# hammershock/3dgs-avatar-release

Measured on AMD Instinct MI355X. Metric: render fps (fwd+bwd) @200k Gaussians 1024x1024 SH3, higher is better.
Workload: dtype f32; 1 GPU; config3: 200k Gaussians, 1024x1024, SH deg 3, forward+backward; shs+scales+rotations inputs, L1 loss (L1 fused into the rasterizer: l1_target); tile_rect=1, l1=fused, long_lists=0, gaussians=200000, width=1024, height=1024, sh_degree=3, frames_per_rank=1857, total_frames=1857, ranks=1, backend=none, parallelism=frames sharded x1

## Files before the change

3dgs-avatar-release_amd/csrc/capi.hip:

```cpp
#include "common.h"
#include <string.h>
#include <stdlib.h>
#include <atomic>

static thread_local int g_last_hip = 0;
static thread_local const char* g_last_stage = "";
void gs_set_error(int hip_err, const char* stage) {
    g_last_hip = hip_err;
    g_last_stage = stage;
}

static std::atomic<int> g_tune[GS_TUNE_COUNT] = {};
static bool g_tune_init = false;
static void tune_defaults() {
    if (g_tune_init) return;
    g_tune_init = true;
    g_tune[GS_TUNE_XCD_MAP].store(1);
    g_tune[GS_TUNE_DEPTH_SORT].store(1);
    g_tune[GS_TUNE_NT_STORES].store(1);
    g_tune[GS_TUNE_BWD_CHUNKS].store(1);
    g_tune[GS_TUNE_FWD4].store(1);
    if (const char* e = getenv("GSPLAT_FWD4")) g_tune[GS_TUNE_FWD4].store(atoi(e));
    g_tune[GS_TUNE_FWDC_CH].store((int)FWDC_CH_MIN);
    g_tune[GS_TUNE_FWDC_DIV].store((int)FWD4_TOTAL_DIV);
    if (const char* e = getenv("GSPLAT_FWDC_DIV")) { const int v = atoi(e); if (v >= 1) g_tune[GS_TUNE_FWDC_DIV].store(v); }
    if (const char* e = getenv("GSPLAT_FWDC_CH")) { const int v = atoi(e); if (v >= 64 && (v & (v - 1)) == 0) g_tune[GS_TUNE_FWDC_CH].store(v); }
    g_tune[GS_TUNE_SHARED_QLIST].store(1);
    g_tune[GS_TUNE_ONES_FAST].store(1);
    g_tune[GS_TUNE_SMALL_TILES].store(BWD_CHUNK_MAX_TILES);
    g_tune[GS_TUNE_BWD_ORDER].store(1);
    g_tune[GS_TUNE_FWD_MARKS].store(1);
}
int gs_tune_get(int key) {
    tune_defaults();
    return (key >= 0 && key < GS_TUNE_COUNT) ? g_tune[key].load(std::memory_order_relaxed) : 0;
}

#include <vector>
struct ProfRec { const char* name; hipEvent_t a, b; };
struct ProfState {
    bool on = false;
// ... 158 lines not shown

static int forward_phase1(const GsFwdArgs* a, void* geom, size_t geom_bytes, void* img, size_t img_bytes, int32_t* radii,
                          int64_t* count_host_pinned, unsigned long long* poll, void* stream) {
    int rc = validate(a);
    if (rc != GS_OK) return rc;
    if (!geom || !img || (a->P > 0 && !radii)) return GS_E_BAD_ARG;
    const GeomLayout L = geom_layout(a->P);
    const ImgLayout I = img_layout(a->W, a->H, a->long_lists);
    if (geom_bytes < L.total || img_bytes < I.total) return GS_E_WORKSPACE;
    hipStream_t s = (hipStream_t)stream;
    char* g = (char*)geom;
    unsigned long long* count = (unsigned long long*)(g + L.count);
    if (a->P == 0) {
        rc = gs_zero_async(count, 24, "count.zero", s);
        if (rc != GS_OK) return rc;
    } else {
        uint32_t* k0 = (uint32_t*)(g + L.key0);
        uint32_t* k1 = (uint32_t*)(g + L.key1);
        uint32_t* v0 = (uint32_t*)(g + L.val0);
        uint32_t* v1 = (uint32_t*)(g + L.val1);
        ZeroJob zt;
        sort_totals_region((uint32_t*)(g + L.hist), a->P, 32, &zt.ptr, &zt.words);
        const ZeroJob zi{(uint32_t*)((char*)img + I.tile_tot), (int)(I.tile_zero_bytes / 4)};
        { StageScope sc_("preprocess", s);
        rc = launch_preprocess(*a, (float*)(g + L.rec), (float*)(g + L.depths), (uint32_t*)(g + L.tiles),
                               (uint32_t*)(g + L.clamped), k0, v0, radii, (uint32_t*)(g + L.wsum), (uint32_t*)(g + L.wkmin),
                               (uint32_t*)(g + L.wkmax), zt, zi, s); }
        if (rc != GS_OK) return rc;
        if (gs_tune_get(GS_TUNE_DEPTH_SORT)) {
            StageScope sc_("depth_sort", s);
            const DepthSortState st{(unsigned long long*)(g + L.ds_tmp), (unsigned long long*)(g + L.ds_tmp2),
                                    (uint32_t*)(g + L.ds_cnt), (uint32_t*)(g + L.ds_pre),
                                    (uint32_t*)(g + L.ds_tot),
                                    (uint32_t*)(g + L.ds_loc), (uint32_t*)(g + L.ds_grp), (uint32_t*)(g + L.ds_range), L.ds_nb,
                                    L.ds_blocks};
            const PairNumbering pn{(const uint32_t*)(g + L.tiles), (const uint32_t*)(g + L.wsum), (float*)(g + L.rec), count, poll,
                                   (uint32_t*)(g + L.chunk_pairs), (a->P + 255) / 256};
            const RankOut ro{(const float*)(g + L.rec), (const uint32_t*)(g + L.tiles), v0, (uint4*)(g + L.ranklist),
                             (uint32_t*)(g + L.chunk_pairs)};
            rc = launch_depth_sort(k0, (const uint32_t*)(g + L.wkmin), (const uint32_t*)(g + L.wkmax), L.nwaves, a->P, st, pn, ro,
                                   a->debug, s);
            if (rc != GS_OK) return rc;
        } else {
            { StageScope sc_("pair_scan", s);
            rc = launch_first_pair((const uint32_t*)(g + L.tiles), (const uint32_t*)(g + L.wsum), (float*)(g + L.rec), count, poll,
                                   a->P, a->debug, s); }
            if (rc != GS_OK) return rc;
            { StageScope sc_("depth_sort", s);
            rc = launch_sort_pairs(k0, v0, k1, v1, (uint32_t*)(g + L.hist), a->P, 32, true, a->debug, s); }
            if (rc != GS_OK) return rc;
            { StageScope sc_("rank_list", s);
            rc = launch_rank_list(v0, (const float*)(g + L.rec), (const uint32_t*)(g + L.tiles), (uint4*)(g + L.ranklist),
                                  (uint32_t*)(g + L.chunk_pairs), a->P, a->debug, s); }
            if (rc != GS_OK) return rc;
        }
    }
    if (count_host_pinned && (!poll || a->P == 0)) {
        hipError_t e = hipMemcpyAsync(count_host_pinned, count, 8, hipMemcpyDeviceToHost, s);
// ... 616 lines not shown
int gs_tuning(const char* name, int value) {
    if (!name) return GS_E_BAD_ARG;
    tune_defaults();
    if (strcmp(name, "xcd_map") == 0) { g_tune[GS_TUNE_XCD_MAP].store(value); return GS_OK; }
    if (strcmp(name, "small_tiles") == 0) { g_tune[GS_TUNE_SMALL_TILES].store(value); return GS_OK; }
    if (strcmp(name, "ones_fast") == 0) { g_tune[GS_TUNE_ONES_FAST].store(value); return GS_OK; }
    if (strcmp(name, "shared_qlist") == 0) { g_tune[GS_TUNE_SHARED_QLIST].store(value); return GS_OK; }
    if (strcmp(name, "fwd4") == 0) { g_tune[GS_TUNE_FWD4].store(value); return GS_OK; }
    if (strcmp(name, "fwdc_div") == 0) {
        if (value < 1) return GS_E_BAD_ARG;
        g_tune[GS_TUNE_FWDC_DIV].store(value);
        return GS_OK;
    }
    if (strcmp(name, "fwdc_ch") == 0) {
        if (value < 64 || (value & (value - 1)) != 0) return GS_E_BAD_ARG;
        g_tune[GS_TUNE_FWDC_CH].store(value);
        return GS_OK;
    }
    if (strcmp(name, "bwd_chunks") == 0) { g_tune[GS_TUNE_BWD_CHUNKS].store(value); return GS_OK; }
    if (strcmp(name, "nt_stores") == 0) { g_tune[GS_TUNE_NT_STORES].store(value); return GS_OK; }
    if (strcmp(name, "fwd_marks") == 0) { g_tune[GS_TUNE_FWD_MARKS].store(value); return GS_OK; }
    if (strcmp(name, "bwd_order") == 0) { g_tune[GS_TUNE_BWD_ORDER].store(value); return GS_OK; }
    if (strcmp(name, "depth_sort") == 0) { g_tune[GS_TUNE_DEPTH_SORT].store(value); return GS_OK; }
    return GS_E_BAD_ARG;
}

const char* gs_status_string(int code) {
    switch (code) {
        case GS_OK: return "ok";
        case GS_E_BAD_ARG: return "bad argument (null required pointer, non-positive size, unsupported SH degree / more than 16 SH coefficients, or rotations not 16-byte aligned)";
        case GS_E_EXCLUSIVE: return "provide exactly one of shs/colors_precomp and exactly one of (scales, rotations)/cov3D_precomp";
        case GS_E_TOO_LARGE: return "num_rendered or tile grid exceeds the supported index space";
        case GS_E_HIP: return "HIP error";
        case GS_E_WORKSPACE: return "state/workspace buffer smaller than gs_*_bytes requires";
        case GS_E_CAPTURE: return "the stream is being captured into a graph and this call is not capture-safe with these arguments (include/gsplat_mi355.h, \"Stream capture\"); nothing was enqueued";
        default: return "unknown status";
    }
}
int gs_last_hip_error(void) { return g_last_hip; }
const char* gs_last_stage(void) { return g_last_stage; }
const char* gs_build_info(void) { return "gsplat_mi355 gfx950 wave64 tile16 rec48"; }

}
```

3dgs-avatar-release_amd/csrc/common.h:

```cpp
#pragma once
#include <hip/hip_runtime.h>
#include <stdint.h>
#include <stddef.h>
#include "../../include/gsplat_mi355.h"

#define TILE 16
#define WAVE 64
#define REC_F 12
#define GS_MAX_PAIRS 0x3FFFFFFFll

static inline size_t align_up(size_t x, size_t a) { return (x + a - 1) / a * a; }

#define SORT_ITEMS 4096
#define SORT_SMALL_N (1 << 20)
#define SORT_TOTALS_REPL 16
static inline size_t sort_table_words(size_t n) {
    const size_t items = n <= (size_t)SORT_SMALL_N ? 1024 : SORT_ITEMS;
    return (size_t)256 * ((n + items - 1) / items + 4 * SORT_TOTALS_REPL);
}
#define SCAN_ITEMS 2048

#ifndef DS_ITEMS
#define DS_ITEMS 2048
#endif
#ifndef DS_PER_BUCKET
#define DS_PER_BUCKET 64
#endif
static inline int ds_buckets(int P) {
    int nb = (P / DS_PER_BUCKET + 63) / 64 * 64;
    return nb < 256 ? 256 : (nb > 4096 ? 4096 : nb);
}

#define TB_MAX_SEG 64
struct GeomLayout {
    size_t rec, depths, tiles, clamped, key0, key1, val0, val1, ranklist, chunk_pairs, wsum, wkmin, wkmax, hist, count,
        ds_tmp, ds_tmp2, ds_cnt, ds_pre, ds_tot, ds_loc, ds_grp, ds_range, seg_start, total;
    int nblk_sort, nwaves, ds_nb, ds_blocks;
};
static inline GeomLayout geom_layout(int P) {
    GeomLayout L;
    size_t o = 0;
    size_t n = (size_t)(P > 0 ? P : 1);
    auto take = [&](size_t bytes) { size_t at = o; o = align_up(o + bytes, 256); return at; };
    L.nblk_sort = (int)((n + SORT_ITEMS - 1) / SORT_ITEMS);
    L.nwaves = (int)((n + 255) / 256) * 4;
    L.rec = take(n * REC_F * 4);
    L.depths = take(n * 4);
    L.tiles = take(n * 4);
    L.clamped = take(n * 4);
    L.key0 = take(n * 4);
    L.key1 = take(n * 4);
    L.val0 = take(n * 4);
    L.val1 = take(n * 4);
    L.ranklist = take(n * 16);
    L.chunk_pairs = take(((n + 255) / 256) * 4);
    L.wsum = take((size_t)L.nwaves * 4);
    L.wkmin = take((size_t)L.nwaves * 4);
    L.wkmax = take((size_t)L.nwaves * 4);
    L.hist = take(sort_table_words(n) * 4);
    L.count = take(64);
    L.ds_nb = ds_buckets(P);
    L.ds_blocks = (int)((n + DS_ITEMS - 1) / DS_ITEMS);
    L.ds_tmp = take(n * 8);
    L.ds_tmp2 = take(n * 8);
    L.ds_cnt = take((size_t)L.ds_blocks * (L.ds_nb + 1) * 4);
    L.ds_pre = take((size_t)L.ds_blocks * (L.ds_nb + 1) * 4);
    L.ds_tot = take((size_t)(L.ds_nb + 1) * 4);
    L.ds_loc = take((size_t)(L.ds_nb + 1) * 4);
    L.ds_grp = take((size_t)((L.ds_nb + 1 + 63) / 64) * 4);
    L.ds_range = take(16);
    L.seg_start = take((size_t)(TB_MAX_SEG + 2) * 4);
    L.total = o;
    return L;
}

struct BinLayout {
    size_t point_list, qlist, marks, marks_flag, total;
};
static inline BinLayout bin_layout(int64_t D) {
    BinLayout L;
    size_t o = 0;
    size_t n = (size_t)(D > 0 ? D : 1);
    auto take = [&](size_t bytes) { size_t at = o; o = align_up(o + bytes, 256); return at; };
    L.point_list = take(n * 4);
    L.qlist = take(n * 16);
    L.marks = take(n * 16);
    L.marks_flag = take(4);
    L.total = o;
    return L;
}

#define TB_W 64
#ifndef TB_H
#define TB_H 4
#endif
#define TB_TILES (TB_W * TB_H)
struct BinGrid { int nbx, nby, nblocks, nseg_max; };
static inline BinGrid bin_grid(int gx, int gy) {
    BinGrid G;
    G.nbx = (gx + TB_W - 1) / TB_W;
    G.nby = (gy + TB_H - 1) / TB_H;
    G.nblocks = G.nbx * G.nby;
#ifndef TB_TARGET_WGS
#define TB_TARGET_WGS 512
#endif
    int s = (TB_TARGET_WGS + G.nblocks - 1) / G.nblocks;
    G.nseg_max = s < 1 ? 1 : (s > TB_MAX_SEG ? TB_MAX_SEG : s);
    return G;
}
static inline int bin_segments(const BinGrid& G, int P) {
    int s = (P + 1023) / 1024;
    if (s < 1) s = 1;
    return s < G.nseg_max ? s : G.nseg_max;
}

enum { GS_TUNE_XCD_MAP = 0, GS_TUNE_DEPTH_SORT = 1, GS_TUNE_NT_STORES = 2, GS_TUNE_BWD_CHUNKS = 3, GS_TUNE_FWD4 = 4, GS_TUNE_SMALL_TILES = 5, GS_TUNE_SHARED_QLIST = 6, GS_TUNE_ONES_FAST = 7, GS_TUNE_BWD_ORDER = 8, GS_TUNE_FWD_MARKS = 9, GS_TUNE_FWDC_CH = 10, GS_TUNE_FWDC_DIV = 11, GS_TUNE_COUNT = 12 };
int gs_tune_get(int key);

#define BWD_CH 128
#define BWD_KMAX 16
#define BWD_CHUNK_MAX_TILES 2048
#define FWD4_MAX_TILES 2048
#define FWD4_MIN_LIST 512u
#ifndef FWD4_TOTAL_DIV
#define FWD4_TOTAL_DIV 320ull
#endif

#define FWDC_CH_MIN 256u
#define FWDC_SPARSE_PAIRS 524288ull
#define FWDC_MAX_UNITS 4096
#define FWDC_MAX_TILES (FWDC_MAX_UNITS / 2)
#ifdef FWDC_PROF
#define FWDC_SLOTS 9
#else
#define FWDC_SLOTS 8
#endif
#define FWDC_DEAD 0x80000000u
#define FWDC_SPIN_MAX (1 << 16)
struct ImgLayout {
// ... 159 lines not shown
        for (int k = 0; k < 4; k++) {
            const int c = c0 + k0 + k;
            if (k0 + k < per && c < nchunks) {
                const int sgc = segment_of(before, scale, nseg);
                for (int sg = prev_seg + 1; sg <= sgc; sg++) seg_start[sg] = (uint32_t)c;
                prev_seg = sgc;
                before += w[k];
                if (c == nchunks - 1)
                    for (int sg = prev_seg + 1; sg <= nseg; sg++) seg_start[sg] = (uint32_t)nchunks;
            }
        }
    }
}

__device__ __forceinline__ uint32_t xcc_id() {
    uint32_t v;
    asm volatile("s_getreg_b32 %0, hwreg(HW_REG_XCC_ID, 0, 4)" : "=s"(v));
    return v & 7u;
}
__device__ __forceinline__ void zero_job(const ZeroJob z) {
    for (int k = blockIdx.x * blockDim.x + threadIdx.x; k < z.words; k += gridDim.x * blockDim.x) z.ptr[k] = 0u;
}

struct PairCount { const unsigned long long* dev; uint32_t cap; };
__device__ __forceinline__ uint32_t pair_count(const PairCount pc) {
    const unsigned long long d = *pc.dev;
    return d <= (unsigned long long)pc.cap ? (uint32_t)d : 0u;
}


__device__ __forceinline__ void render_block_map(int b, int xmap, int* slot, int* q) {
    if (xmap) {
        *slot = ((b >> 5) << 3) + (b & 7);
        *q = (b >> 3) & 3;
    } else {
        *slot = b >> 2;
        *q = b & 3;
    }
}
static inline bool forward_small_image(int ntiles, int long_lists) { return few_long_lists_mode(ntiles, long_lists) && gs_tune_get(GS_TUNE_FWD4) == 1; }
static inline bool forward_chunked(int ntiles, int long_lists) { return few_long_lists_mode(ntiles, long_lists) && gs_tune_get(GS_TUNE_FWD4) == 2; }
static inline int render_grid_blocks(int ntiles, int xmap) { return xmap ? ((ntiles + 7) / 8) * 32 : ntiles * 4; }

struct StageScope {
    hipStream_t s;
    StageScope(const char* stage, hipStream_t st) : s(st) { gs_prof_begin(stage, st); }
    ~StageScope() { gs_prof_end(s); }
};

int launch_preprocess(const GsFwdArgs& a, float* rec, float* depths, uint32_t* tiles, uint32_t* clamped,
                      uint32_t* sort_keys, uint32_t* sort_vals, int32_t* radii, uint32_t* wave_tiles, uint32_t* wave_kmin,
                      uint32_t* wave_kmax, ZeroJob zero, ZeroJob zero2, hipStream_t s);
struct DepthSortState { unsigned long long *tmp, *tmp2; uint32_t *cnt, *pre, *tot, *loc, *grp, *range; int nb, blocks; };
struct PairNumbering { const uint32_t *tiles, *wave_tiles; float* rec; unsigned long long *count, *host_count; uint32_t* chunk_pairs; int nchunks; };
struct RankOut { const float* rec; const uint32_t* tiles; uint32_t* sorted_idx; uint4* ranklist; uint32_t* chunk_pairs; };
int launch_depth_sort(const uint32_t* keys, const uint32_t* wave_kmin, const uint32_t* wave_kmax, int nwaves, int P,
                      DepthSortState st, PairNumbering pn, RankOut ro, int debug, hipStream_t s);
struct CopyJob { const uint32_t* src; uint32_t* dst; int words; };
struct SecondOnes {
    const float* src_final_T; const uint32_t* src_n_contrib; const uint32_t* src_ncon_c; const uint32_t* src_qcount;
    const float4* src_ckpt; const uint32_t* src_ck_start;
    float* out_color; float* final_T; uint32_t* n_contrib; uint32_t* ncon_c; uint32_t* qcount; float4* ckpt; uint32_t* ck_start;
    const float* bg; int W, H, gx, ntiles, chunks;
};
__device__ __forceinline__ void second_ones_body(const SecondOnes& A, const int block, const int pixel_blocks) {
    if (block < pixel_blocks) {
        const size_t HW = (size_t)A.H * A.W, pid = (size_t)block * 256 + threadIdx.x;
        if (pid < HW) {
            const float Tf = A.src_final_T[pid];
            A.final_T[pid] = Tf;
            A.n_contrib[pid] = A.src_n_contrib[pid];
            A.ncon_c[pid] = A.src_ncon_c[pid];
            A.out_color[pid] = (1.0f - Tf) + Tf * A.bg[0];
            A.out_color[HW + pid] = (1.0f - Tf) + Tf * A.bg[1];
            A.out_color[2 * HW + pid] = (1.0f - Tf) + Tf * A.bg[2];
        }
// ... 148 lines not shown
```

3dgs-avatar-release_amd/csrc/depth_sort.hip:

```cpp
#include "common.h"

#define DS_THREADS 256
#define DS_WAVE_CAP 1024
#define DS_WG_BUCKETS 4
#define DS_CAP_BIG (DS_WG_BUCKETS * DS_WAVE_CAP)

__device__ __forceinline__ unsigned long long ds_bucket_scale(unsigned long long span, int nb) {
    return ((unsigned long long)nb << 32) / span;
}
__device__ __forceinline__ uint32_t ds_bucket_of(uint32_t key, uint32_t kmin, unsigned long long scale, int nb) {
    if (key == 0xFFFFFFFFu || key < kmin) return (uint32_t)nb;
    const uint32_t d = key - kmin;
    const uint32_t lo = (uint32_t)scale, hi = (uint32_t)(scale >> 32);
    const uint32_t b = __umulhi(d, lo) + d * hi;
    return b < (uint32_t)nb ? b : (uint32_t)(nb - 1);
}

#define DS_WAVE_WORDS 16
__global__ __launch_bounds__(DS_THREADS) void ds_count_kernel(const uint32_t* __restrict__ keys,
                                                              const uint32_t* __restrict__ wave_kmin,
                                                              const uint32_t* __restrict__ wave_kmax, int nwaves, int P,
                                                              int nb, uint32_t* __restrict__ cnt,
                                                              uint32_t* __restrict__ krange, const PairNumbering pn) {
    extern __shared__ uint32_t s_hist[];
    __shared__ uint32_t s_red[8];
    __shared__ unsigned long long s_before[DS_THREADS / 64];
    __shared__ uint32_t s_wave[DS_ITEMS / 64 + 1];
    const int tid = threadIdx.x, lane = tid & 63, wid = tid >> 6;
    constexpr int WPB = DS_ITEMS / 64;
    constexpr int NU = DS_ITEMS / DS_THREADS;
    static_assert(WPB <= 64, "one wave scans the workgroup's wave sums");
    static_assert(DS_THREADS == 256, "four partial sums");
    const int w0 = WPB * (int)blockIdx.x;
    const uint32_t* __restrict__ tiles = pn.tiles;
    const uint32_t* __restrict__ wave_tiles = pn.wave_tiles;
    uint32_t k[NU], tv[NU];
#pragma unroll
    for (int u = 0; u < NU; u++) {
        const int i = blockIdx.x * DS_ITEMS + u * DS_THREADS + tid;
        k[u] = i < P ? keys[i] : 0u;
        tv[u] = i < P ? tiles[i] : 0u;
    }
    const uint32_t own = (wid == 0 && lane < WPB && w0 + lane < nwaves) ? wave_tiles[w0 + lane] : 0u;
    uint32_t lo = 0xFFFFFFFFu, hi = 0u;
    unsigned long long before = 0;
    for (int base = 0; base < nwaves; base += DS_THREADS * DS_WAVE_WORDS) {
        uint32_t a[DS_WAVE_WORDS], c[DS_WAVE_WORDS], t[DS_WAVE_WORDS];
#pragma unroll
        for (int u = 0; u < DS_WAVE_WORDS; u++) {
            const int w = base + u * DS_THREADS + tid;
            a[u] = w < nwaves ? wave_kmin[w] : 0xFFFFFFFFu;
            c[u] = w < nwaves ? wave_kmax[w] : 0u;
            t[u] = w < w0 ? wave_tiles[w] : 0u;
        }
#pragma unroll
        for (int u = 0; u < DS_WAVE_WORDS; u++) {
            lo = min(lo, a[u]);
            hi = max(hi, c[u]);
            before += t[u];
        }
    }
    for (int c = blockIdx.x * DS_THREADS + tid; c < pn.nchunks; c += gridDim.x * DS_THREADS) pn.chunk_pairs[c] = 0u;
    for (int b = tid; b <= nb; b += DS_THREADS) s_hist[b] = 0u;
    lo = wave_min(lo);
    hi = wave_max(hi);
    before = wave_sum(before);
    if (lane == 0) { s_red[wid] = lo; s_red[4 + wid] = hi; s_before[wid] = before; }
    if (wid == 0) {
        const uint32_t x = wave_scan_incl(own);
        if (lane < WPB) s_wave[lane] = x - own;
        if (lane == 63) s_wave[WPB] = x;
    }
    __syncthreads();
    const uint32_t kmin = min(min(s_red[0], s_red[1]), min(s_red[2], s_red[3]));
    const uint32_t kmax = max(max(s_red[4], s_red[5]), max(s_red[6], s_red[7]));
    const unsigned long long span = kmax >= kmin ? (unsigned long long)(kmax - kmin) + 1ull : 1ull;
    const unsigned long long block_base = (s_before[0] + s_before[1]) + (s_before[2] + s_before[3]);
    const unsigned long long scale = ds_bucket_scale(span, nb);
    if (blockIdx.x == 0 && tid == 0) {
        krange[0] = kmin;
        krange[1] = (uint32_t)scale;
        krange[2] = (uint32_t)(scale >> 32);
    }
    if (blockIdx.x == gridDim.x - 1 && tid == 0) {
        const unsigned long long total = block_base + s_wave[WPB];
        pn.count[0] = total;
        pn.count[2] = 0ull;
        if (pn.host_count) __hip_atomic_store(pn.host_count, total, __ATOMIC_RELAXED, __HIP_MEMORY_SCOPE_SYSTEM);
    }
#pragma unroll
    for (int u = 0; u < NU; u++) {
        const int i = blockIdx.x * DS_ITEMS + u * DS_THREADS + tid;
        const uint32_t x = wave_scan_incl(tv[u]);
        if (i < P) {
            pn.rec[(size_t)i * REC_F + 9] = __uint_as_float((uint32_t)block_base + s_wave[u * (DS_THREADS / 64) + wid] + x - tv[u]);
            atomicAdd(&s_hist[ds_bucket_of(k[u], kmin, scale, nb)], 1u);
        }
    }
    __syncthreads();
    for (int b = tid; b <= nb; b += DS_THREADS) cnt[(size_t)blockIdx.x * (nb + 1) + b] = s_hist[b];
}

#define DSP_ROWS 32
__global__ __launch_bounds__(256) void ds_prefix_kernel(const uint32_t* __restrict__ cnt, uint32_t* __restrict__ pre,
                                                        uint32_t* __restrict__ tot, uint32_t* __restrict__ loc,
                                                        uint32_t* __restrict__ grp, int nbp, int blocks) {
    __shared__ uint32_t s_part[4][64];
    const int lane = threadIdx.x & 63, wid = threadIdx.x >> 6;
    const int b = blockIdx.x * 64 + lane;
    const bool live = b < nbp;
    const int per = (blocks + 3) >> 2, r0 = wid * per, r1 = min(blocks, r0 + per);
    const bool one_trip = per <= DSP_ROWS;
    uint32_t v[DSP_ROWS];
    uint32_t sum = 0;
    for (int g0 = r0; g0 < r1; g0 += DSP_ROWS) {
#pragma unroll
        for (int u = 0; u < DSP_ROWS; u++) v[u] = (live && g0 + u < r1) ? cnt[(size_t)(g0 + u) * nbp + b] : 0u;
#pragma unroll
        for (int u = 0; u < DSP_ROWS; u++) sum += v[u];
    }
    s_part[wid][lane] = sum;
    __syncthreads();
    uint32_t acc = 0, total = 0;
#pragma unroll
    for (int w = 0; w < 4; w++) {
        const uint32_t q = s_part[w][lane];
        if (w < wid) acc += q;
        total += q;
    }
    for (int g0 = r0; g0 < r1; g0 += DSP_ROWS) {
        if (!one_trip) {
#pragma unroll
            for (int u = 0; u < DSP_ROWS; u++) v[u] = (live && g0 + u < r1) ? cnt[(size_t)(g0 + u) * nbp + b] : 0u;
        }
#pragma unroll
        for (int u = 0; u < DSP_ROWS; u++) {
            if (live && g0 + u < r1) pre[(size_t)(g0 + u) * nbp + b] = acc;
            acc += v[u];
        }
    }
    if (wid == 0) {
        if (live) tot[b] = total;
        const uint32_t x = wave_scan_incl(live ? total : 0u);
        if (live) loc[b] = x - total;
        if (lane == 63) grp[blockIdx.x] = x;
    }
}

#define DS_MAX_NBP 4097
__global__ __launch_bounds__(DS_THREADS) void ds_scatter_kernel(const uint32_t* __restrict__ keys,
                                                                const uint32_t* __restrict__ krange, int P,
                                                                int nb, const uint32_t* __restrict__ cnt,
                                                                const uint32_t* __restrict__ loc,
                                                                const uint32_t* __restrict__ grp,
                                                                unsigned long long* __restrict__ tmp) {
    extern __shared__ uint32_t s_mem[];
    const int nbp = nb + 1;
    uint32_t* s_next = s_mem;
    uint32_t* s_grp = s_mem + nbp;
    const int tid = threadIdx.x;
    constexpr int NB_T = (DS_MAX_NBP + DS_THREADS - 1) / DS_THREADS;
    uint32_t k[DS_ITEMS / DS_THREADS], first[NB_T];
#pragma unroll
    for (int u = 0; u < DS_ITEMS / DS_THREADS; u++) {
        const int i = blockIdx.x * DS_ITEMS + u * DS_THREADS + tid;
        k[u] = i < P ? keys[i] : 0u;
    }
#pragma unroll
    for (int u = 0; u < NB_T; u++) {
        const int b = u * DS_THREADS + tid;
        first[u] = b < nbp ? loc[b] + cnt[(size_t)blockIdx.x * nbp + b] : 0u;
    }
    const int ngrp = (nbp + 63) / 64;
    if (tid < 64) {
        uint32_t x = 0, carry = 0;
        for (int g0 = 0; g0 < ngrp; g0 += 64) {
            const uint32_t v = g0 + tid < ngrp ? grp[g0 + tid] : 0u;
            x = wave_scan_incl(v);
            if (g0 + tid < ngrp) s_grp[g0 + tid] = carry + x - v;
            carry += (uint32_t)__builtin_amdgcn_readlane((int)x, 63);
        }
    }
    const uint32_t kmin = krange[0];
    const unsigned long long scale = (unsigned long long)krange[1] | ((unsigned long long)krange[2] << 32);
    __syncthreads();
#pragma unroll
    for (int u = 0; u < NB_T; u++) {
        const int b = u * DS_THREADS + tid;
        if (b < nbp) s_next[b] = s_grp[b >> 6] + first[u];
    }
    __syncthreads();
#pragma unroll
    for (int u = 0; u < DS_ITEMS / DS_THREADS; u++) {
        const int i = blockIdx.x * DS_ITEMS + u * DS_THREADS + tid;
        if (i < P) {
            const uint32_t pos = atomicAdd(&s_next[ds_bucket_of(k[u], kmin, scale, nb)], 1u);
            tmp[pos] = ((unsigned long long)k[u] << 32) | (unsigned long long)(uint32_t)i;
        }
    }
}

template <typename LOAD, typename STORE, typename SYNC>
__device__ __forceinline__ void ds_bitonic(const long long n, LOAD load, STORE store, SYNC sync) {
    long long n_pad = 2;
    while (n_pad < n) n_pad <<= 1;
    const long long half = n_pad >> 1;
    for (long long k = 2, lk = 0; k <= n_pad; k <<= 1, lk++) {
        for (long long t = threadIdx.x; t < half; t += DS_THREADS) {
            const long long blk = t >> lk, off = t & ((k >> 1) - 1);
            const long long i = blk * k + off, p = blk * k + (k - 1 - off);
            if (p < n) {
                const unsigned long long a = load(i), c = load(p);
                if (a > c) { store(i, c); store(p, a); }
            }
        }
        sync();
        for (long long j = k >> 2; j > 0; j >>= 1) {
            for (long long t = threadIdx.x; t < half; t += DS_THREADS) {
                const long long i = ((t & ~(j - 1)) << 1) | (t & (j - 1)), p = i + j;
// ... 256 lines not shown
        start = wave_sum(part) + in_group;
    }
    const bool large = n > DS_WAVE_CAP;
    if (lane == 0) {
        s_large[wid][0] = large ? (uint32_t)n : 0u;
        s_large[wid][1] = start;
    }
    if (n > 0 && !large) ds_wave_bucket(tmp + start, s + wid * DS_WAVE_CAP, n, start, ro);
    __syncthreads();
    for (int w = 0; w < DS_WG_BUCKETS; w++) {
        const int nl = (int)s_large[w][0];
        if (nl) {
            if (nl > DS_CAP_BIG) ds_giant_bucket(tmp + s_large[w][1], tmp2 + s_large[w][1], s, s_sub, nl, s_large[w][1], ro);
            else ds_large_bucket(tmp + s_large[w][1], s, nl, s_large[w][1], ro);
            __syncthreads();
        }
    }
}

int launch_depth_sort(const uint32_t* keys, const uint32_t* wave_kmin, const uint32_t* wave_kmax, int nwaves, int P,
                      DepthSortState st, PairNumbering pn, RankOut ro, int debug, hipStream_t s) {
    const int nbp = st.nb + 1;
    if (nbp > DS_MAX_NBP) return GS_E_BAD_ARG;
    const size_t lds_count = (size_t)nbp * 4, lds_scatter = (size_t)(nbp + 66) * 4;
    hipLaunchKernelGGL(ds_count_kernel, dim3(st.blocks), dim3(DS_THREADS), lds_count, s, keys, wave_kmin, wave_kmax, nwaves, P,
                       st.nb, st.cnt, st.range, pn);
    GS_LAUNCH_CHECK("depth_sort.count", debug, s);
    hipLaunchKernelGGL(ds_prefix_kernel, dim3((nbp + 63) / 64), dim3(256), 0, s, st.cnt, st.pre, st.tot, st.loc, st.grp, nbp,
                       st.blocks);
    GS_LAUNCH_CHECK("depth_sort.prefix", debug, s);
    hipLaunchKernelGGL(ds_scatter_kernel, dim3(st.blocks), dim3(DS_THREADS), lds_scatter, s, keys, st.range, P, st.nb, st.pre,
                       st.loc, st.grp, st.tmp);
    GS_LAUNCH_CHECK("depth_sort.scatter", debug, s);
    const int helpers = P / 4096 < 1 ? 1 : (P / 4096 > 128 ? 128 : P / 4096);
    hipLaunchKernelGGL(ds_bucket_sort_kernel, dim3((st.nb + DS_WG_BUCKETS - 1) / DS_WG_BUCKETS + helpers), dim3(DS_THREADS), 0, s,
                       st.tmp, st.tmp2, st.tot, st.loc, st.grp, st.nb, ro);
    GS_LAUNCH_CHECK("depth_sort.buckets", debug, s);
    return GS_OK;
}
```

3dgs-avatar-release_amd/csrc/preprocess.hip:

```cpp
#include "common.h"
#include "gs_math.h"

__device__ __forceinline__ float3 load_and_eval_sh(int deg, int M, const float3 p, const float3 campos,
                                                   const float* __restrict__ shs, int i, uint32_t* clamped) {
    const float* g = shs + (size_t)i * M * 3;
    if (M == 16 && ((uintptr_t)shs & 15u) == 0) {
        float l[48];
        const float4* g4 = reinterpret_cast<const float4*>(g);
#pragma unroll
        for (int k = 0; k < 12; k++) {
            const float4 v = g4[k];
            l[4 * k] = v.x; l[4 * k + 1] = v.y; l[4 * k + 2] = v.z; l[4 * k + 3] = v.w;
        }
        return sh_to_rgb(deg, p, campos, l, clamped);
    }
    return sh_to_rgb(deg, p, campos, g, clamped);
}

__global__ __launch_bounds__(256) void preprocess_kernel(
    int P, int deg, int M, const float* __restrict__ means3D, const float* __restrict__ scales,
    float scale_modifier, const float* __restrict__ rotations, const float* __restrict__ opacities,
    const float* __restrict__ shs, const float* __restrict__ colors_precomp, const float* __restrict__ cov3D_precomp,
    const float* __restrict__ viewmatrix, const float* __restrict__ projmatrix, const float* __restrict__ campos,
    int W, int H, float tanfovx, float tanfovy, float focal_x, float focal_y, int gx, int gy, int tile_rect,
    float* __restrict__ rec, float* __restrict__ depths, uint32_t* __restrict__ tiles, uint32_t* __restrict__ clamped,
    uint32_t* __restrict__ sort_keys, uint32_t* __restrict__ sort_vals, int32_t* __restrict__ radii,
    uint32_t* __restrict__ wave_tiles, uint32_t* __restrict__ wave_kmin, uint32_t* __restrict__ wave_kmax, ZeroJob zero,
    ZeroJob zero2) {
    zero_job(zero);
    zero_job(zero2);
    const int gi = blockIdx.x * blockDim.x + threadIdx.x;
    const bool live = gi < P;
    const int i = live ? gi : P - 1;

    float V[16], PV[16];
#pragma unroll
    for (int k = 0; k < 16; k++) { V[k] = viewmatrix[k]; PV[k] = projmatrix[k]; }

    float4 r0 = make_float4(0.f, 0.f, 0.f, 0.f), r1 = r0;
    float r2x = 0.f;
    uint32_t off_bits = 0, rmin_bits = 0, rsize_bits = 0, cl = 0, tt = 0;
    float depth = 0.f;
    int radius = 0;

    const float3 p = make_float3(means3D[3 * i], means3D[3 * i + 1], means3D[3 * i + 2]);
    float c6in[6] = {0.f, 0.f, 0.f, 0.f, 0.f, 0.f};
    float3 sc_in = make_float3(0.f, 0.f, 0.f);
    float4 q_in = make_float4(1.f, 0.f, 0.f, 0.f);
    if (cov3D_precomp) {
#pragma unroll
        for (int k = 0; k < 6; k++) c6in[k] = cov3D_precomp[6 * i + k];
// ... 84 lines not shown
    if (live) {
        float4* R = reinterpret_cast<float4*>(rec) + (size_t)i * 3;
        R[0] = r0;
        R[1] = r1;
        R[2] = make_float4(r2x, __uint_as_float(off_bits), __uint_as_float(rmin_bits), __uint_as_float(rsize_bits));
        depths[i] = depth;
        tiles[i] = tt;
        clamped[i] = cl;
        radii[i] = radius;
        sort_keys[i] = tt ? __float_as_uint(depth) : 0xFFFFFFFFu;
        sort_vals[i] = (uint32_t)i;
    }
    uint32_t wsum = live ? tt : 0u;
    const bool keyed = live && tt != 0u;
    uint32_t kmin = keyed ? __float_as_uint(depth) : 0xFFFFFFFFu, kmax = keyed ? __float_as_uint(depth) : 0u;
    wsum = wave_sum(wsum);
    kmin = wave_min(kmin);
    kmax = wave_max(kmax);
    if ((threadIdx.x & 63) == 0) {
        wave_tiles[gi >> 6] = wsum;
        wave_kmin[gi >> 6] = kmin;
        wave_kmax[gi >> 6] = kmax;
    }
}

int launch_preprocess(const GsFwdArgs& a, float* rec, float* depths, uint32_t* tiles, uint32_t* clamped,
                      uint32_t* sort_keys, uint32_t* sort_vals, int32_t* radii, uint32_t* wave_tiles, uint32_t* wave_kmin,
                      uint32_t* wave_kmax, ZeroJob zero, ZeroJob zero2, hipStream_t s) {
    const int gx = (a.W + TILE - 1) / TILE, gy = (a.H + TILE - 1) / TILE;
    const float focal_y = a.H / (2.0f * a.tanfovy), focal_x = a.W / (2.0f * a.tanfovx);
    const int blocks = (a.P + 255) / 256;
    hipLaunchKernelGGL(preprocess_kernel, dim3(blocks), dim3(256), 0, s, a.P, a.sh_degree, a.M, a.means3D, a.scales,
                       a.scale_modifier, a.rotations, a.opacities, a.shs, a.colors_precomp, a.cov3D_precomp,
                       a.viewmatrix, a.projmatrix, a.campos, a.W, a.H, a.tanfovx, a.tanfovy, focal_x, focal_y, gx, gy,
                       a.tile_rect,
                       rec, depths, tiles, clamped, sort_keys, sort_vals, radii, wave_tiles, wave_kmin, wave_kmax, zero, zero2);
    GS_LAUNCH_CHECK("preprocess", a.debug, s);
    return GS_OK;
}

__global__ __launch_bounds__(256) void recolor_kernel(int P, int deg, int M, const float* __restrict__ means3D,
                                                      const float* __restrict__ shs,
                                                      const float* __restrict__ colors_precomp,
                                                      const float* __restrict__ campos,
                                                      const float4* __restrict__ rec_src,
                                                      const uint32_t* __restrict__ tiles_src,
                                                      float4* __restrict__ rec_dst, uint32_t* __restrict__ tiles_dst,
                                                      uint32_t* __restrict__ clamped_dst,
                                                      unsigned long long* __restrict__ not_ones, const CopyJob c0,
                                                      const CopyJob c1, const ZeroJob z0, const int recolor_blocks, const SecondOnes ones,
                                                      const int pixel_blocks) {
    if ((int)blockIdx.x >= recolor_blocks) {
        second_ones_body(ones, (int)blockIdx.x - recolor_blocks, pixel_blocks);
        return;
    }
    const int i = blockIdx.x * blockDim.x + threadIdx.x;
    for (int k = i; k < c0.words; k += recolor_blocks * (int)blockDim.x) c0.dst[k] = c0.src[k];
    for (int k = i; k < c1.words; k += recolor_blocks * (int)blockDim.x) c1.dst[k] = c1.src[k];
    for (int k = i; k < z0.words; k += recolor_blocks * (int)blockDim.x) z0.ptr[k] = 0u;
// ... 62 lines not shown
```

Baseline: 1720 frames/s.

## Fuse depth-sort bucket counting into preprocess using previous frame's key range

Removes the separate depth-sort count kernel. Preprocess now builds each block's bucket histogram in shared memory, using the depth range stored from the previous call (validated by a tag, padded, with a fixed fallback range). The per-row pair bases and the global key range are computed by an extra block of the prefix kernel, and per-Gaussian pair numbering moves into the scatter kernel. Preprocess blocks grow to DS_ITEMS (now 1024) threads so each block maps to one count row. This saves a launch and a read pass over the keys, but bucket balance now depends on the previous frame's range, and the larger blocks may change occupancy.

```diff
diff --git a/3dgs-avatar-release_amd/csrc/capi.hip b/3dgs-avatar-release_amd/csrc/capi.hip
--- a/3dgs-avatar-release_amd/csrc/capi.hip
+++ b/3dgs-avatar-release_amd/csrc/capi.hip
@@ -17,6 +17,8 @@
     g_tune_init = true;
     g_tune[GS_TUNE_XCD_MAP].store(1);
     g_tune[GS_TUNE_DEPTH_SORT].store(1);
+    g_tune[GS_TUNE_DS_MAP].store(1);
+    if (const char* e = getenv("GSPLAT_DS_MAP")) g_tune[GS_TUNE_DS_MAP].store(atoi(e));
     g_tune[GS_TUNE_NT_STORES].store(1);
     g_tune[GS_TUNE_BWD_CHUNKS].store(1);
     g_tune[GS_TUNE_FWD4].store(1);
@@ -221,18 +223,21 @@
         ZeroJob zt;
         sort_totals_region((uint32_t*)(g + L.hist), a->P, 32, &zt.ptr, &zt.words);
         const ZeroJob zi{(uint32_t*)((char*)img + I.tile_tot), (int)(I.tile_zero_bytes / 4)};
+        const bool bucket_sort = gs_tune_get(GS_TUNE_DEPTH_SORT) != 0;
+        const DsCount dc{(uint32_t*)(g + L.ds_range), bucket_sort ? (uint32_t*)(g + L.ds_cnt) : nullptr, L.ds_nb,
+                         gs_tune_get(GS_TUNE_DS_MAP) == 0 ? 1 : 0};
         { StageScope sc_("preprocess", s);
         rc = launch_preprocess(*a, (float*)(g + L.rec), (float*)(g + L.depths), (uint32_t*)(g + L.tiles),
                                (uint32_t*)(g + L.clamped), k0, v0, radii, (uint32_t*)(g + L.wsum), (uint32_t*)(g + L.wkmin),
-                               (uint32_t*)(g + L.wkmax), zt, zi, s); }
+                               (uint32_t*)(g + L.wkmax), zt, zi, dc, s); }
         if (rc != GS_OK) return rc;
-        if (gs_tune_get(GS_TUNE_DEPTH_SORT)) {
+        if (bucket_sort) {
             StageScope sc_("depth_sort", s);
             const DepthSortState st{(unsigned long long*)(g + L.ds_tmp), (unsigned long long*)(g + L.ds_tmp2),
                                     (uint32_t*)(g + L.ds_cnt), (uint32_t*)(g + L.ds_pre),
                                     (uint32_t*)(g + L.ds_tot),
-                                    (uint32_t*)(g + L.ds_loc), (uint32_t*)(g + L.ds_grp), (uint32_t*)(g + L.ds_range), L.ds_nb,
-                                    L.ds_blocks};
+                                    (uint32_t*)(g + L.ds_loc), (uint32_t*)(g + L.ds_grp), (uint32_t*)(g + L.ds_range),
+                                    (uint32_t*)(g + L.ds_base), L.ds_nb, L.ds_blocks};
             const PairNumbering pn{(const uint32_t*)(g + L.tiles), (const uint32_t*)(g + L.wsum), (float*)(g + L.rec), count, poll,
                                    (uint32_t*)(g + L.chunk_pairs), (a->P + 255) / 256};
             const RankOut ro{(const float*)(g + L.rec), (const uint32_t*)(g + L.tiles), v0, (uint4*)(g + L.ranklist),
@@ -895,6 +900,7 @@
     if (strcmp(name, "fwd_marks") == 0) { g_tune[GS_TUNE_FWD_MARKS].store(value); return GS_OK; }
     if (strcmp(name, "bwd_order") == 0) { g_tune[GS_TUNE_BWD_ORDER].store(value); return GS_OK; }
     if (strcmp(name, "depth_sort") == 0) { g_tune[GS_TUNE_DEPTH_SORT].store(value); return GS_OK; }
+    if (strcmp(name, "ds_map") == 0) { g_tune[GS_TUNE_DS_MAP].store(value); return GS_OK; }
     return GS_E_BAD_ARG;
 }
 
diff --git a/3dgs-avatar-release_amd/csrc/common.h b/3dgs-avatar-release_amd/csrc/common.h
--- a/3dgs-avatar-release_amd/csrc/common.h
+++ b/3dgs-avatar-release_amd/csrc/common.h
@@ -21,7 +21,7 @@
 #define SCAN_ITEMS 2048
 
 #ifndef DS_ITEMS
-#define DS_ITEMS 2048
+#define DS_ITEMS 1024
 #endif
 #ifndef DS_PER_BUCKET
 #define DS_PER_BUCKET 64
@@ -34,7 +34,7 @@
 #define TB_MAX_SEG 64
 struct GeomLayout {
     size_t rec, depths, tiles, clamped, key0, key1, val0, val1, ranklist, chunk_pairs, wsum, wkmin, wkmax, hist, count,
-        ds_tmp, ds_tmp2, ds_cnt, ds_pre, ds_tot, ds_loc, ds_grp, ds_range, seg_start, total;
+        ds_tmp, ds_tmp2, ds_cnt, ds_pre, ds_tot, ds_loc, ds_grp, ds_range, ds_base, seg_start, total;
     int nblk_sort, nwaves, ds_nb, ds_blocks;
 };
 static inline GeomLayout geom_layout(int P) {
@@ -43,7 +43,7 @@
     size_t n = (size_t)(P > 0 ? P : 1);
     auto take = [&](size_t bytes) { size_t at = o; o = align_up(o + bytes, 256); return at; };
     L.nblk_sort = (int)((n + SORT_ITEMS - 1) / SORT_ITEMS);
-    L.nwaves = (int)((n + 255) / 256) * 4;
+    L.nwaves = (int)((n + DS_ITEMS - 1) / DS_ITEMS) * (DS_ITEMS / 64);
     L.rec = take(n * REC_F * 4);
     L.depths = take(n * 4);
     L.tiles = take(n * 4);
@@ -68,7 +68,8 @@
     L.ds_tot = take((size_t)(L.ds_nb + 1) * 4);
     L.ds_loc = take((size_t)(L.ds_nb + 1) * 4);
     L.ds_grp = take((size_t)((L.ds_nb + 1 + 63) / 64) * 4);
-    L.ds_range = take(16);
+    L.ds_range = take(32);
+    L.ds_base = take((size_t)L.ds_blocks * 4);
     L.seg_start = take((size_t)(TB_MAX_SEG + 2) * 4);
     L.total = o;
     return L;
@@ -114,7 +115,7 @@
     return s < G.nseg_max ? s : G.nseg_max;
 }
 
-enum { GS_TUNE_XCD_MAP = 0, GS_TUNE_DEPTH_SORT = 1, GS_TUNE_NT_STORES = 2, GS_TUNE_BWD_CHUNKS = 3, GS_TUNE_FWD4 = 4, GS_TUNE_SMALL_TILES = 5, GS_TUNE_SHARED_QLIST = 6, GS_TUNE_ONES_FAST = 7, GS_TUNE_BWD_ORDER = 8, GS_TUNE_FWD_MARKS = 9, GS_TUNE_FWDC_CH = 10, GS_TUNE_FWDC_DIV = 11, GS_TUNE_COUNT = 12 };
+enum { GS_TUNE_XCD_MAP = 0, GS_TUNE_DEPTH_SORT = 1, GS_TUNE_NT_STORES = 2, GS_TUNE_BWD_CHUNKS = 3, GS_TUNE_FWD4 = 4, GS_TUNE_SMALL_TILES = 5, GS_TUNE_SHARED_QLIST = 6, GS_TUNE_ONES_FAST = 7, GS_TUNE_BWD_ORDER = 8, GS_TUNE_FWD_MARKS = 9, GS_TUNE_FWDC_CH = 10, GS_TUNE_FWDC_DIV = 11, GS_TUNE_DS_MAP = 12, GS_TUNE_COUNT = 13 };
 int gs_tune_get(int key);
 
 #define BWD_CH 128
@@ -320,6 +321,33 @@
     for (int k = blockIdx.x * blockDim.x + threadIdx.x; k < z.words; k += gridDim.x * blockDim.x) z.ptr[k] = 0u;
 }
 
+#define DS_PAD_SHIFT 5
+#define DS_RANGE_TAG 0x6b5d3a17u
+#define DS_FIXED_KMIN 0x3E4CCCCDu
+#define DS_FIXED_KMAX 0x454CCCCDu
+struct DsMap { uint32_t kmin, kmax; unsigned long long scale; };
+__device__ __forceinline__ DsMap ds_map_make(uint32_t kmin, uint32_t kmax, int nb) {
+    DsMap m;
+    m.kmin = kmin;
+    m.kmax = kmax;
+    m.scale = ((unsigned long long)nb << 32) / ((unsigned long long)(kmax - kmin) + 1ull);
+    return m;
+}
+__device__ __forceinline__ DsMap ds_map_stored(uint32_t lo, uint32_t hi, uint32_t tag, int nb, bool fixed) {
+    if (fixed || lo > hi || tag != (lo ^ hi ^ DS_RANGE_TAG)) return ds_map_make(DS_FIXED_KMIN, DS_FIXED_KMAX, nb);
+    const uint32_t pad = (hi - lo) >> DS_PAD_SHIFT;
+    return ds_map_make(lo > pad ? lo - pad : 0u, hi < 0xFFFFFFFFu - pad ? hi + pad : 0xFFFFFFFFu, nb);
+}
+__device__ __forceinline__ uint32_t ds_bucket_of(uint32_t key, const DsMap& m, int nb) {
+    if (key == 0xFFFFFFFFu) return (uint32_t)nb;
+    if (key <= m.kmin) return 0u;
+    if (key >= m.kmax) return (uint32_t)(nb - 1);
+    const uint32_t d = key - m.kmin;
+    const uint32_t lo = (uint32_t)m.scale, hi = (uint32_t)(m.scale >> 32);
+    const uint32_t b = __umulhi(d, lo) + d * hi;
+    return b < (uint32_t)nb ? b : (uint32_t)(nb - 1);
+}
+
 struct PairCount { const unsigned long long* dev; uint32_t cap; };
 __device__ __forceinline__ uint32_t pair_count(const PairCount pc) {
     const unsigned long long d = *pc.dev;
@@ -346,10 +374,11 @@
     ~StageScope() { gs_prof_end(s); }
 };
 
+struct DsCount { uint32_t* range; uint32_t* cnt; int nb, fixed_map; };
 int launch_preprocess(const GsFwdArgs& a, float* rec, float* depths, uint32_t* tiles, uint32_t* clamped,
                       uint32_t* sort_keys, uint32_t* sort_vals, int32_t* radii, uint32_t* wave_tiles, uint32_t* wave_kmin,
-                      uint32_t* wave_kmax, ZeroJob zero, ZeroJob zero2, hipStream_t s);
-struct DepthSortState { unsigned long long *tmp, *tmp2; uint32_t *cnt, *pre, *tot, *loc, *grp, *range; int nb, blocks; };
+                      uint32_t* wave_kmax, ZeroJob zero, ZeroJob zero2, DsCount dc, hipStream_t s);
+struct DepthSortState { unsigned long long *tmp, *tmp2; uint32_t *cnt, *pre, *tot, *loc, *grp, *range, *base; int nb, blocks; };
 struct PairNumbering { const uint32_t *tiles, *wave_tiles; float* rec; unsigned long long *count, *host_count; uint32_t* chunk_pairs; int nchunks; };
 struct RankOut { const float* rec; const uint32_t* tiles; uint32_t* sorted_idx; uint4* ranklist; uint32_t* chunk_pairs; };
 int launch_depth_sort(const uint32_t* keys, const uint32_t* wave_kmin, const uint32_t* wave_kmax, int nwaves, int P,
diff --git a/3dgs-avatar-release_amd/csrc/depth_sort.hip b/3dgs-avatar-release_amd/csrc/depth_sort.hip
--- a/3dgs-avatar-release_amd/csrc/depth_sort.hip
+++ b/3dgs-avatar-release_amd/csrc/depth_sort.hip
@@ -5,109 +5,72 @@
 #define DS_WG_BUCKETS 4
 #define DS_CAP_BIG (DS_WG_BUCKETS * DS_WAVE_CAP)
 
-__device__ __forceinline__ unsigned long long ds_bucket_scale(unsigned long long span, int nb) {
-    return ((unsigned long long)nb << 32) / span;
-}
-__device__ __forceinline__ uint32_t ds_bucket_of(uint32_t key, uint32_t kmin, unsigned long long scale, int nb) {
-    if (key == 0xFFFFFFFFu || key < kmin) return (uint32_t)nb;
-    const uint32_t d = key - kmin;
-    const uint32_t lo = (uint32_t)scale, hi = (uint32_t)(scale >> 32);
-    const uint32_t b = __umulhi(d, lo) + d * hi;
-    return b < (uint32_t)nb ? b : (uint32_t)(nb - 1);
-}
-
-#define DS_WAVE_WORDS 16
-__global__ __launch_bounds__(DS_THREADS) void ds_count_kernel(const uint32_t* __restrict__ keys,
-                                                              const uint32_t* __restrict__ wave_kmin,
-                                                              const uint32_t* __restrict__ wave_kmax, int nwaves, int P,
-                                                              int nb, uint32_t* __restrict__ cnt,
-                                                              uint32_t* __restrict__ krange, const PairNumbering pn) {
-    extern __shared__ uint32_t s_hist[];
-    __shared__ uint32_t s_red[8];
-    __shared__ unsigned long long s_before[DS_THREADS / 64];
-    __shared__ uint32_t s_wave[DS_ITEMS / 64 + 1];
+#define DSP_ROWS 64
+struct DsSide { const uint32_t *wave_kmin, *wave_kmax; int nwaves; uint32_t *range, *base; PairNumbering pn; };
+
+__device__ __forceinline__ void ds_side_job(const DsSide& sd, int rows) {
+    __shared__ unsigned long long s_w[4];
+    __shared__ uint32_t s_lo[4], s_hi[4];
+    constexpr int WPR = DS_ITEMS / 64;
     const int tid = threadIdx.x, lane = tid & 63, wid = tid >> 6;
-    constexpr int WPB = DS_ITEMS / 64;
-    constexpr int NU = DS_ITEMS / DS_THREADS;
-    static_assert(WPB <= 64, "one wave scans the workgroup's wave sums");
-    static_assert(DS_THREADS == 256, "four partial sums");
-    const int w0 = WPB * (int)blockIdx.x;
-    const uint32_t* __restrict__ tiles = pn.tiles;
-    const uint32_t* __restrict__ wave_tiles = pn.wave_tiles;
-    uint32_t k[NU], tv[NU];
-#pragma unroll
-    for (int u = 0; u < NU; u++) {
-        const int i = blockIdx.x * DS_ITEMS + u * DS_THREADS + tid;
-        k[u] = i < P ? keys[i] : 0u;
-        tv[u] = i < P ? tiles[i] : 0u;
-    }
-    const uint32_t own = (wid == 0 && lane < WPB && w0 + lane < nwaves) ? wave_tiles[w0 + lane] : 0u;
+    const PairNumbering& pn = sd.pn;
+    for (int c = tid; c < pn.nchunks; c += 256) pn.chunk_pairs[c] = 0u;
     uint32_t lo = 0xFFFFFFFFu, hi = 0u;
-    unsigned long long before = 0;
-    for (int base = 0; base < nwaves; base += DS_THREADS * DS_WAVE_WORDS) {
-        uint32_t a[DS_WAVE_WORDS], c[DS_WAVE_WORDS], t[DS_WAVE_WORDS];
-#pragma unroll
-        for (int u = 0; u < DS_WAVE_WORDS; u++) {
-            const int w = base + u * DS_THREADS + tid;
-            a[u] = w < nwaves ? wave_kmin[w] : 0xFFFFFFFFu;
-            c[u] = w < nwaves ? wave_kmax[w] : 0u;
-            t[u] = w < w0 ? wave_tiles[w] : 0u;
-        }
-#pragma unroll
-        for (int u = 0; u < DS_WAVE_WORDS; u++) {
+    unsigned long long carry = 0;
+    for (int r0 = 0; r0 < rows; r0 += 256) {
+        const int r = r0 + tid;
+        const bool ok = r < rows;
+        uint32_t a[WPR], c[WPR], t[WPR];
+#pragma unroll
+        for (int u = 0; u < WPR; u++) {
+            const int w = r * WPR + u;
+            a[u] = ok ? sd.wave_kmin[w] : 0xFFFFFFFFu;
+            c[u] = ok ? sd.wave_kmax[w] : 0u;
+            t[u] = ok ? pn.wave_tiles[w] : 0u;
+        }
+        unsigned long long sum = 0;
+#pragma unroll
+        for (int u = 0; u < WPR; u++) {
             lo = min(lo, a[u]);
             hi = max(hi, c[u]);
-            before += t[u];
-        }
-    }
-    for (int c = blockIdx.x * DS_THREADS + tid; c < pn.nchunks; c += gridDim.x * DS_THREADS) pn.chunk_pairs[c] = 0u;
-    for (int b = tid; b <= nb; b += DS_THREADS) s_hist[b] = 0u;
+            sum += t[u];
+        }
+        const unsigned long long x = wave_scan_incl(sum);
+        if (lane == 63) s_w[wid] = x;
+        __syncthreads();
+        unsigned long long before = carry + (x - sum);
+        for (int w = 0; w < wid; w++) before += s_w[w];
+        if (ok) sd.base[r] = (uint32_t)before;
+        carry += (s_w[0] + s_w[1]) + (s_w[2] + s_w[3]);
+        __syncthreads();
+    }
     lo = wave_min(lo);
     hi = wave_max(hi);
-    before = wave_sum(before);
-    if (lane == 0) { s_red[wid] = lo; s_red[4 + wid] = hi; s_before[wid] = before; }
-    if (wid == 0) {
-        const uint32_t x = wave_scan_incl(own);
-        if (lane < WPB) s_wave[lane] = x - own;
-        if (lane == 63) s_wave[WPB] = x;
-    }
-    __syncthreads();
-    const uint32_t kmin = min(min(s_red[0], s_red[1]), min(s_red[2], s_red[3]));
-    const uint32_t kmax = max(max(s_red[4], s_red[5]), max(s_red[6], s_red[7]));
-    const unsigned long long span = kmax >= kmin ? (unsigned long long)(kmax - kmin) + 1ull : 1ull;
-    const unsigned long long block_base = (s_before[0] + s_before[1]) + (s_before[2] + s_before[3]);
-    const unsigned long long scale = ds_bucket_scale(span, nb);
-    if (blockIdx.x == 0 && tid == 0) {
-        krange[0] = kmin;
-        krange[1] = (uint32_t)scale;
-        krange[2] = (uint32_t)(scale >> 32);
-    }
-    if (blockIdx.x == gridDim.x - 1 && tid == 0) {
-        const unsigned long long total = block_base + s_wave[WPB];
-        pn.count[0] = total;
+    if (lane == 0) { s_lo[wid] = lo; s_hi[wid] = hi; }
+    __syncthreads();
+    if (tid == 0) {
+        lo = min(min(s_lo[0], s_lo[1]), min(s_lo[2], s_lo[3]));
+        hi = max(max(s_hi[0], s_hi[1]), max(s_hi[2], s_hi[3]));
+        sd.range[4] = lo;
+        sd.range[5] = hi;
+        sd.range[6] = lo ^ hi ^ DS_RANGE_TAG;
+        pn.count[0] = carry;
         pn.count[2] = 0ull;
-        if (pn.host_count) __hip_atomic_store(pn.host_count, total, __ATOMIC_RELAXED, __HIP_MEMORY_SCOPE_SYSTEM);
-    }
-#pragma unroll
-    for (int u = 0; u < NU; u++) {
-        const int i = blockIdx.x * DS_ITEMS + u * DS_THREADS + tid;
-        const uint32_t x = wave_scan_incl(tv[u]);
-        if (i < P) {
-            pn.rec[(size_t)i * REC_F + 9] = __uint_as_float((uint32_t)block_base + s_wave[u * (DS_THREADS / 64) + wid] + x - tv[u]);
-            atomicAdd(&s_hist[ds_bucket_of(k[u], kmin, scale, nb)], 1u);
-        }
-    }
-    __syncthreads();
-    for (int b = tid; b <= nb; b += DS_THREADS) cnt[(size_t)blockIdx.x * (nb + 1) + b] = s_hist[b];
-}
-
-#define DSP_ROWS 32
+        if (pn.host_count) __hip_atomic_store(pn.host_count, carry, __ATOMIC_RELAXED, __HIP_MEMORY_SCOPE_SYSTEM);
+    }
+}
+
 __global__ __launch_bounds__(256) void ds_prefix_kernel(const uint32_t* __restrict__ cnt, uint32_t* __restrict__ pre,
                                                         uint32_t* __restrict__ tot, uint32_t* __restrict__ loc,
-                                                        uint32_t* __restrict__ grp, int nbp, int blocks) {
+                                                        uint32_t* __restrict__ grp, int nbp, int blocks, const DsSide sd) {
+    if (blockIdx.x == 0) {
+        ds_side_job(sd, blocks);
+        return;
+    }
     __shared__ uint32_t s_part[4][64];
     const int lane = threadIdx.x & 63, wid = threadIdx.x >> 6;
-    const int b = blockIdx.x * 64 + lane;
+    const int gb = (int)blockIdx.x - 1;
+    const int b = gb * 64 + lane;
     const bool live = b < nbp;
     const int per = (blocks + 3) >> 2, r0 = wid * per, r1 = min(blocks, r0 + per);
     const bool one_trip = per <= DSP_ROWS;
@@ -143,34 +106,46 @@
         if (live) tot[b] = total;
         const uint32_t x = wave_scan_incl(live ? total : 0u);
         if (live) loc[b] = x - total;
-        if (lane == 63) grp[blockIdx.x] = x;
+        if (lane == 63) grp[gb] = x;
     }
 }
 
 #define DS_MAX_NBP 4097
 __global__ __launch_bounds__(DS_THREADS) void ds_scatter_kernel(const uint32_t* __restrict__ keys,
-                                                                const uint32_t* __restrict__ krange, int P,
+                                                                const uint32_t* __restrict__ range, int P,
                                                                 int nb, const uint32_t* __restrict__ cnt,
                                                                 const uint32_t* __restrict__ loc,
                                                                 const uint32_t* __restrict__ grp,
-                                                                unsigned long long* __restrict__ tmp) {
+                                                                unsigned long long* __restrict__ tmp,
+                                                                const uint32_t* __restrict__ base, const PairNumbering pn) {
     extern __shared__ uint32_t s_mem[];
+    __shared__ uint32_t s_wave[DS_ITEMS / 64];
     const int nbp = nb + 1;
     uint32_t* s_next = s_mem;
     uint32_t* s_grp = s_mem + nbp;
-    const int tid = threadIdx.x;
+    const int tid = threadIdx.x, lane = tid & 63, wid = tid >> 6;
+    constexpr int NU = DS_ITEMS / DS_THREADS;
+    constexpr int WPR = DS_ITEMS / 64;
+    static_assert(WPR <= 64, "one wave scans the row's wave sums");
     constexpr int NB_T = (DS_MAX_NBP + DS_THREADS - 1) / DS_THREADS;
-    uint32_t k[DS_ITEMS / DS_THREADS], first[NB_T];
-#pragma unroll
-    for (int u = 0; u < DS_ITEMS / DS_THREADS; u++) {
+    uint32_t k[NU], tv[NU], first[NB_T];
+#pragma unroll
+    for (int u = 0; u < NU; u++) {
         const int i = blockIdx.x * DS_ITEMS + u * DS_THREADS + tid;
         k[u] = i < P ? keys[i] : 0u;
+        tv[u] = i < P ? pn.tiles[i] : 0u;
     }
 #pragma unroll
     for (int u = 0; u < NB_T; u++) {
         const int b = u * DS_THREADS + tid;
         first[u] = b < nbp ? loc[b] + cnt[(size_t)blockIdx.x * nbp + b] : 0u;
     }
+    const uint32_t own = (wid == 0 && lane < WPR) ? pn.wave_tiles[blockIdx.x * WPR + lane] : 0u;
+    const uint32_t row_base = base[blockIdx.x];
+    DsMap m;
+    m.kmin = range[0];
+    m.kmax = range[1];
+    m.scale = (unsigned long long)range[2] | ((unsigned long long)range[3] << 32);
     const int ngrp = (nbp + 63) / 64;
     if (tid < 64) {
         uint32_t x = 0, carry = 0;
@@ -180,9 +155,9 @@
             if (g0 + tid < ngrp) s_grp[g0 + tid] = carry + x - v;
             carry += (uint32_t)__builtin_amdgcn_readlane((int)x, 63);
         }
-    }
-    const uint32_t kmin = krange[0];
-    const unsigned long long scale = (unsigned long long)krange[1] | ((unsigned long long)krange[2] << 32);
+        const uint32_t y = wave_scan_incl(own);
+        if (lane < WPR) s_wave[lane] = y - own;
+    }
     __syncthreads();
 #pragma unroll
     for (int u = 0; u < NB_T; u++) {
@@ -191,10 +166,12 @@
     }
     __syncthreads();
 #pragma unroll
-    for (int u = 0; u < DS_ITEMS / DS_THREADS; u++) {
+    for (int u = 0; u < NU; u++) {
         const int i = blockIdx.x * DS_ITEMS + u * DS_THREADS + tid;
+        const uint32_t x = wave_scan_incl(tv[u]);
         if (i < P) {
-            const uint32_t pos = atomicAdd(&s_next[ds_bucket_of(k[u], kmin, scale, nb)], 1u);
+            pn.rec[(size_t)i * REC_F + 9] = __uint_as_float(row_base + s_wave[u * (DS_THREADS / 64) + wid] + x - tv[u]);
+            const uint32_t pos = atomicAdd(&s_next[ds_bucket_of(k[u], m, nb)], 1u);
             tmp[pos] = ((unsigned long long)k[u] << 32) | (unsigned long long)(uint32_t)i;
         }
     }
@@ -497,15 +474,14 @@
                       DepthSortState st, PairNumbering pn, RankOut ro, int debug, hipStream_t s) {
     const int nbp = st.nb + 1;
     if (nbp > DS_MAX_NBP) return GS_E_BAD_ARG;
-    const size_t lds_count = (size_t)nbp * 4, lds_scatter = (size_t)(nbp + 66) * 4;
-    hipLaunchKernelGGL(ds_count_kernel, dim3(st.blocks), dim3(DS_THREADS), lds_count, s, keys, wave_kmin, wave_kmax, nwaves, P,
-                       st.nb, st.cnt, st.range, pn);
-    GS_LAUNCH_CHECK("depth_sort.count", debug, s);
-    hipLaunchKernelGGL(ds_prefix_kernel, dim3((nbp + 63) / 64), dim3(256), 0, s, st.cnt, st.pre, st.tot, st.loc, st.grp, nbp,
-                       st.blocks);
+    if (nwaves < st.blocks * (DS_ITEMS / 64)) return GS_E_BAD_ARG;
+    const size_t lds_scatter = (size_t)(nbp + 66) * 4;
+    const DsSide sd{wave_kmin, wave_kmax, nwaves, st.range, st.base, pn};
+    hipLaunchKernelGGL(ds_prefix_kernel, dim3(1 + (nbp + 63) / 64), dim3(256), 0, s, st.cnt, st.pre, st.tot, st.loc, st.grp, nbp,
+                       st.blocks, sd);
     GS_LAUNCH_CHECK("depth_sort.prefix", debug, s);
     hipLaunchKernelGGL(ds_scatter_kernel, dim3(st.blocks), dim3(DS_THREADS), lds_scatter, s, keys, st.range, P, st.nb, st.pre,
-                       st.loc, st.grp, st.tmp);
+                       st.loc, st.grp, st.tmp, st.base, pn);
     GS_LAUNCH_CHECK("depth_sort.scatter", debug, s);
     const int helpers = P / 4096 < 1 ? 1 : (P / 4096 > 128 ? 128 : P / 4096);
     hipLaunchKernelGGL(ds_bucket_sort_kernel, dim3((st.nb + DS_WG_BUCKETS - 1) / DS_WG_BUCKETS + helpers), dim3(DS_THREADS), 0, s,
diff --git a/3dgs-avatar-release_amd/csrc/preprocess.hip b/3dgs-avatar-release_amd/csrc/preprocess.hip
--- a/3dgs-avatar-release_amd/csrc/preprocess.hip
+++ b/3dgs-avatar-release_amd/csrc/preprocess.hip
@@ -17,7 +17,9 @@
     return sh_to_rgb(deg, p, campos, g, clamped);
 }
 
-__global__ __launch_bounds__(256) void preprocess_kernel(
+#define PP_THREADS DS_ITEMS
+static_assert(PP_THREADS <= 1024 && PP_THREADS % 64 == 0, "one workgroup per count row");
+__global__ __launch_bounds__(PP_THREADS) void preprocess_kernel(
     int P, int deg, int M, const float* __restrict__ means3D, const float* __restrict__ scales,
     float scale_modifier, const float* __restrict__ rotations, const float* __restrict__ opacities,
     const float* __restrict__ shs, const float* __restrict__ colors_precomp, const float* __restrict__ cov3D_precomp,
@@ -26,7 +28,16 @@
     float* __restrict__ rec, float* __restrict__ depths, uint32_t* __restrict__ tiles, uint32_t* __restrict__ clamped,
     uint32_t* __restrict__ sort_keys, uint32_t* __restrict__ sort_vals, int32_t* __restrict__ radii,
     uint32_t* __restrict__ wave_tiles, uint32_t* __restrict__ wave_kmin, uint32_t* __restrict__ wave_kmax, ZeroJob zero,
-    ZeroJob zero2) {
+    ZeroJob zero2, const DsCount dc) {
+    extern __shared__ uint32_t s_hist[];
+    const bool count = dc.cnt != nullptr;
+    uint32_t rlo = 0u, rhi = 0u, rtag = 0u;
+    if (count) {
+        rlo = dc.range[4];
+        rhi = dc.range[5];
+        rtag = dc.range[6];
+        for (int b = threadIdx.x; b <= dc.nb; b += PP_THREADS) s_hist[b] = 0u;
+    }
     zero_job(zero);
     zero_job(zero2);
     const int gi = blockIdx.x * blockDim.x + threadIdx.x;
@@ -157,19 +168,34 @@
         wave_kmin[gi >> 6] = kmin;
         wave_kmax[gi >> 6] = kmax;
     }
+    if (count) {
+        const DsMap m = ds_map_stored(rlo, rhi, rtag, dc.nb, dc.fixed_map != 0);
+        if (blockIdx.x == 0 && threadIdx.x == 0) {
+            dc.range[0] = m.kmin;
+            dc.range[1] = m.kmax;
+            dc.range[2] = (uint32_t)m.scale;
+            dc.range[3] = (uint32_t)(m.scale >> 32);
+        }
+        __syncthreads();
+        if (live) atomicAdd(&s_hist[ds_bucket_of(tt ? __float_as_uint(depth) : 0xFFFFFFFFu, m, dc.nb)], 1u);
+        __syncthreads();
+        uint32_t* __restrict__ row = dc.cnt + (size_t)blockIdx.x * (dc.nb + 1);
+        for (int b = threadIdx.x; b <= dc.nb; b += PP_THREADS) row[b] = s_hist[b];
+    }
 }
 
 int launch_preprocess(const GsFwdArgs& a, float* rec, float* depths, uint32_t* tiles, uint32_t* clamped,
                       uint32_t* sort_keys, uint32_t* sort_vals, int32_t* radii, uint32_t* wave_tiles, uint32_t* wave_kmin,
-                      uint32_t* wave_kmax, ZeroJob zero, ZeroJob zero2, hipStream_t s) {
+                      uint32_t* wave_kmax, ZeroJob zero, ZeroJob zero2, DsCount dc, hipStream_t s) {
     const int gx = (a.W + TILE - 1) / TILE, gy = (a.H + TILE - 1) / TILE;
     const float focal_y = a.H / (2.0f * a.tanfovy), focal_x = a.W / (2.0f * a.tanfovx);
-    const int blocks = (a.P + 255) / 256;
-    hipLaunchKernelGGL(preprocess_kernel, dim3(blocks), dim3(256), 0, s, a.P, a.sh_degree, a.M, a.means3D, a.scales,
+    const int blocks = (a.P + PP_THREADS - 1) / PP_THREADS;
+    const size_t lds = dc.cnt ? (size_t)(dc.nb + 1) * 4 : 0;
+    hipLaunchKernelGGL(preprocess_kernel, dim3(blocks), dim3(PP_THREADS), lds, s, a.P, a.sh_degree, a.M, a.means3D, a.scales,
                        a.scale_modifier, a.rotations, a.opacities, a.shs, a.colors_precomp, a.cov3D_precomp,
                        a.viewmatrix, a.projmatrix, a.campos, a.W, a.H, a.tanfovx, a.tanfovy, focal_x, focal_y, gx, gy,
                        a.tile_rect,
-                       rec, depths, tiles, clamped, sort_keys, sort_vals, radii, wave_tiles, wave_kmin, wave_kmax, zero, zero2);
+                       rec, depths, tiles, clamped, sort_keys, sort_vals, radii, wave_tiles, wave_kmin, wave_kmax, zero, zero2, dc);
     GS_LAUNCH_CHECK("preprocess", a.debug, s);
     return GS_OK;
 }
```

After: 1739 frames/s, median of 6. 1.1% higher.
